# ebiggers/libdeflate

Hardware: NVIDIA H100
Metric: MB/s compress+decompress (batched 64 KiB chunks) (higher is better)
Workload: dtype u8

## Files before the change

### libdeflate_b200/csrc/deflate_block.cuh

```cuda
#pragma once

struct lz_group {
	u32 tid, lane, warp, gw, gt;
	__device__ __forceinline__ void sync() const
	{
		if (gt < LZ_THREADS) LDB_BAR_SYNC(LZ_BAR_P, gt);
		else __syncthreads();
	}
};

__constant__ u8 lz_precode_perm[DEFLATE_NUM_PRECODE_SYMS] = {16, 17, 18, 0, 8, 7, 9, 6, 10, 5, 11, 4, 12, 3, 13, 2, 14, 1, 15};

__device__ __forceinline__ u32 lz_static_litlen_len(u32 sym) { return sym < 144 ? 8 : (sym < 256 ? 9 : (sym < 280 ? 7 : 8)); }

__device__ __forceinline__ u32 lz_warp_incl_scan(u32 x, u32 lane)
{
	for (int o2 = 1; o2 < 32; o2 <<= 1) {
		const u32 t = __shfl_up_sync(LDB_FULL_MASK, x, o2);
		if (lane >= (u32)o2) x += t;
	}
	return x;
}

__device__ __forceinline__ u32 lz_group_excl_scan(const lz_group &g, u32 *escan, u32 x, u32 &total)
{
	const u32 incl = lz_warp_incl_scan(x, g.lane);
	if (g.lane == 31) escan[g.warp] = incl;
	g.sync();
	if (g.warp == 0) {
		const u32 y = g.lane < g.gw ? escan[g.lane] : 0;
		const u32 yi = lz_warp_incl_scan(y, g.lane);
		if (g.lane < g.gw) escan[32 + g.lane] = yi - y;
		if (g.lane == g.gw - 1) escan[64] = yi;
	}
	g.sync();
	total = escan[64];
	return escan[32 + g.warp] + (incl - x);
}

struct lz_out {
	u8 *out;
	size_t avail;
	u64 obit;
};

__device__ __forceinline__ void lz_stage_or(u32 *stage, u32 rel_bit, u64 bits, u32 nbits)
{
	if (!nbits) return;
	u32 w = rel_bit >> 5, sh = rel_bit & 31;
	atomicOr(&stage[w], (u32)(bits << sh));
	if (sh + nbits > 32) {
		u64 rest = bits >> (32 - sh);
		atomicOr(&stage[w + 1], (u32)rest);
		if (sh + nbits > 64) atomicOr(&stage[w + 2], (u32)(rest >> 32));
	}
}

__device__ __forceinline__ void lz_stage_reset(const lz_group &g, u32 *stage, const lz_out &o, const u32 *carry)
{
	for (u32 k = g.tid; k < LZ_STAGE_WORDS; k += g.gt) stage[k] = 0;
	g.sync();
	if (g.tid == 0) {
		u32 wv = 0;
		if (carry) {
			wv = *carry;
		} else {
			const u8 *wp = o.out + (o.obit >> 5) * 4;
			for (u32 k = 0; k < (u32)((o.obit >> 3) & 3); k++) wv |= (u32)(*(volatile const u8 *)(wp + k)) << (8 * k);
		}
		stage[0] = wv;
	}
	g.sync();
}

__device__ __forceinline__ void lz_stage_store(const lz_group &g, const u32 *stage, u8 *out, u64 w0, u64 end)
{
	const u64 begin = w0 * 4;
	for (u64 k = begin + g.tid; k < end; k += g.gt) {
		const u32 rel = (u32)(k - begin);
		out[k] = (u8)(stage[rel >> 2] >> (8 * (rel & 3)));
	}
}

__device__ __forceinline__ void lz_flush_words(const lz_out &o, const u32 *stage, u64 first_word, u32 nwords, u32 nthreads)
{
	if ((((uintptr_t)o.out) & 3) == 0) {
		u32 *dst = (u32 *)o.out + first_word;
		for (u32 i = threadIdx.x; i < nwords; i += nthreads) dst[i] = stage[i];
	} else {
		u8 *dst = o.out + first_word * 4;
		for (u32 i = threadIdx.x; i < nwords * 4; i += nthreads) dst[i] = (u8)(stage[i >> 2] >> (8 * (i & 3)));
	}
}

__device__ __forceinline__ void lz_huffman_merge(u32 *nodefreq, u16 *parent, u32 nused)
{
	const u32 INF = 0xffffffffu;
	u32 leaf = 0, inode = nused, nn = nused;
	u32 l0 = nodefreq[0], l1 = nused > 1 ? nodefreq[1] : INF;
	u32 n0 = INF, n1 = INF;
	while (nn < 2 * nused - 1) {
		u32 a, b, fa, fb;
		if (l0 <= n0) { a = leaf++; fa = l0; l0 = l1; l1 = leaf + 1 < nused ? nodefreq[leaf + 1] : INF; }
		else { a = inode++; fa = n0; n0 = n1; n1 = INF; }
		if (n0 == INF && inode < nn) n0 = nodefreq[inode];
		if (l0 <= n0) { b = leaf++; fb = l0; l0 = l1; l1 = leaf + 1 < nused ? nodefreq[leaf + 1] : INF; }
		else { b = inode++; fb = n0; n0 = n1; n1 = INF; }
		const u32 sum = fa + fb;
		nodefreq[nn] = sum;
		parent[a] = (u16)nn;
		parent[b] = (u16)nn;
		nn++;
		if (n0 == INF && inode < nn) n0 = inode == nn - 1 ? sum : nodefreq[inode];
		if (n1 == INF && inode + 1 < nn) n1 = inode + 1 == nn - 1 ? sum : nodefreq[inode + 1];
	}
}

#define LZ_SM_CNT    (LZ_SM_GEXIT + 256)
#define LZ_SM_PFREQ  (LZ_SM_GEXIT)
#define LZ_SM_PLENS  (LZ_SM_GEXIT + 128)
#define LZ_SM_PCODES (LZ_SM_GEXIT + 160)

__device__ __forceinline__ void lz_canonical_codes(const lz_group &g, u8 *sm)
{
	const u8 *lens = sm + LZ_SM_LENS;
	u16 *codes = (u16 *)(sm + LZ_SM_CODES);
	const u32 tid = g.tid;
	if (tid < 320) {
		const u32 l = lens[tid];
		u32 code = 0;
		if (l) {
			const u32 lo = tid < 288 ? 0 : 288;
			const u32 *cn = (u32 *)(sm + LZ_SM_CNT) + (tid < 288 ? 0 : 17);
			u32 first = 0;
			for (u32 k = 1; k < l; k++) first = (first + cn[k]) << 1;
			u32 same = 0;
			for (u32 t = lo; t < tid; t++) same += lens[t] == l;
			code = __brev(first + same) >> (32 - l);
		}
		codes[tid] = (u16)code;
	}
	g.sync();
}

__device__ __forceinline__ void lz_build_codes(const lz_group &g, u8 *sm)
{
	lz_vars *v = (lz_vars *)(sm + LZ_SM_VARS);
	u32 *freq = (u32 *)(sm + LZ_SM_FREQ);
	u8 *lens = sm + LZ_SM_LENS;
	u16 *hsorted = (u16 *)(sm + LZ_SM_R);
	u32 *hnodefreq = (u32 *)(sm + LZ_SM_R + 1024);
	u16 *hparent = (u16 *)(sm + LZ_SM_R + 1024 + 2304);
	u16 *osorted = (u16 *)(sm + LZ_SM_R + 4608);
	u32 *onodefreq = (u32 *)(sm + LZ_SM_R + 4608 + 128);
	u16 *oparent = (u16 *)(sm + LZ_SM_R + 4608 + 128 + 512);
	u32 *hcount = (u32 *)(sm + LZ_SM_CNT), *ocount = hcount + 17;
	const u32 tid = g.tid;
	const bool is_lit = tid < 288;
	const u32 lo = is_lit ? 0 : 288, hi = is_lit ? 288 : 320;
	if (tid == 0) { freq[256] = 1; v->nused_lit = 0; v->nused_off = 0; v->huff_over = 0; }
	if (tid < 34) hcount[tid] = 0;
	g.sync();
	u32 myrank = 0xffffffffu;
	if (tid < 320) {
		const u32 f = freq[tid];
		lens[tid] = 0;
		if (f) {
			u32 rank = 0;
			for (u32 t = lo; t < hi; t++) {
				u32 ft = freq[t];
				rank += (ft != 0) && (ft < f || (ft == f && t < tid));
			}
			myrank = rank;
			(is_lit ? hsorted : osorted)[rank] = (u16)(tid - lo);
			(is_lit ? hnodefreq : onodefreq)[rank] = f;
			atomicAdd(is_lit ? &v->nused_lit : &v->nused_off, 1u);
		}
	}
	g.sync();
	const u32 nused = is_lit ? v->nused_lit : v->nused_off;
	if (tid == 0 && nused >= 2) lz_huffman_merge(hnodefreq, hparent, nused);
	if (tid == 32) { const u32 nu = v->nused_off; if (nu >= 2) lz_huffman_merge(onodefreq, oparent, nu); }
	g.sync();
	if (tid < 320 && myrank != 0xffffffffu && nused >= 2) {
		const u16 *par = is_lit ? hparent : oparent;
		const u32 root = 2 * nused - 2;
		u32 node = myrank, d = 0;
		while (node != root && d <= 15) { node = par[node]; d++; }
		if (d > 15) { d = 15; v->huff_over = 1; }
		atomicAdd(&(is_lit ? hcount : ocount)[d], 1u);
	}
	g.sync();
	if ((tid == 0 || tid == 288) && nused < 2) {
		u8 *ln = lens + lo;
		u32 *cn = is_lit ? hcount : ocount;
		if (nused == 0) { ln[0] = 1; ln[1] = 1; }
		else { const u32 sy = (is_lit ? hsorted : osorted)[0]; ln[sy] = 1; ln[sy ? 0 : 1] = 1; }
		cn[1] = 2;
	}
	if ((tid == 0 || tid == 32) && v->huff_over) {
		u32 *cn = tid == 0 ? hcount : ocount;
		u32 kraft = 0;
		for (u32 l = 1; l <= 15; l++) kraft += cn[l] << (15 - l);
		while (kraft > (1u << 15)) {
			u32 l = 14;
			while (cn[l] == 0) l--;
			cn[l]--;
			cn[l + 1] += 2;
			cn[15]--;
			kraft -= 1;
		}
	}
	g.sync();
	if (tid < 320 && myrank != 0xffffffffu && nused >= 2) {
		const u32 *cn = is_lit ? hcount : ocount;
		u32 cum = 0, len = 1;
		for (u32 l = 15; l >= 1; l--) {
			cum += cn[l];
			if (myrank < cum) { len = l; break; }
		}
		lens[tid] = (u8)len;
	}
	g.sync();
	lz_canonical_codes(g, sm);
}

__device__ __forceinline__ void lz_precode(const lz_group &g, u8 *sm)
{
	lz_vars *v = (lz_vars *)(sm + LZ_SM_VARS);
	const u8 *lens = sm + LZ_SM_LENS;
	u16 *items = (u16 *)(sm + LZ_SM_ITEMS);
	u32 *escan = (u32 *)(sm + LZ_SM_ESCAN);
	u32 *pfreq_sm = (u32 *)(sm + LZ_SM_PFREQ);
	u8 *plens_sm = sm + LZ_SM_PLENS;
	u16 *pcodes_sm = (u16 *)(sm + LZ_SM_PCODES);
	const u32 tid = g.tid, lane = g.lane, warp = g.warp;
	if (tid == 0) {
		u32 hlit = 288;
		while (hlit > 257 && lens[hlit - 1] == 0) hlit--;
		v->hlit = hlit;
	}
	if (tid == 32) {
		u32 hdist = 32;
		while (hdist > 1 && lens[288 + hdist - 1] == 0) hdist--;
		v->hdist = hdist;
	}
	if (tid >= 64 && tid < 64 + 19) pfreq_sm[tid - 64] = 0;
	g.sync();
	{
		const u32 hlit = v->hlit, total = hlit + v->hdist;
		const u32 j = tid;
		const bool inb = j < total;
		const u32 val = inb ? (j < hlit ? lens[j] : lens[288 + j - hlit]) : 0xff;
		const u32 prv = (inb && j > 0) ? (j - 1 < hlit ? lens[j - 1] : lens[288 + j - 1 - hlit]) : 0xfe;
		const bool isstart = inb && val != prv;
		const u32 smask = __ballot_sync(LDB_FULL_MASK, isstart);
		if (lane == 0 && warp < 10) escan[66 + warp] = smask;
		g.sync();
		u32 run = 0, cnt = 0;
		if (isstart) {
			u32 nxt = total;
			u32 m = lane == 31 ? 0 : (smask & ~((2u << lane) - 1));
			if (m) nxt = warp * 32 + __ffs(m) - 1;
			else {
				for (u32 w = warp + 1; w < 10; w++) {
					u32 mm = escan[66 + w];
					if (mm) { nxt = w * 32 + __ffs(mm) - 1; break; }
				}
			}
			run = nxt - j;
			if (val == 0) {
				u32 rem = run % 138;
				cnt = run / 138 + (rem >= 3 ? 1 : rem);
			} else if (run >= 4) {
				u32 rem = (run - 1) % 6;
				cnt = 1 + (run - 1) / 6 + (rem >= 3 ? 1 : rem);
			} else cnt = run;
		}
		u32 ntot;
		const u32 off = lz_group_excl_scan(g, escan, cnt, ntot);
		if (isstart) {
			u32 ni = off;
			if (val == 0) {
				while (run >= 11) {
					u32 r = run < 138 ? run : 138;
					items[ni++] = (u16)(18 | ((r - 11) << 5));
					atomicAdd(&pfreq_sm[18], 1u);
					run -= r;
				}
				if (run >= 3) {
					items[ni++] = (u16)(17 | ((run - 3) << 5));
					atomicAdd(&pfreq_sm[17], 1u);
					run = 0;
				}
			} else if (run >= 4) {
				items[ni++] = (u16)val;
				atomicAdd(&pfreq_sm[val], 1u);
				run--;
				while (run >= 3) {
					u32 r = run < 6 ? run : 6;
					items[ni++] = (u16)(16 | ((r - 3) << 5));
					atomicAdd(&pfreq_sm[16], 1u);
					run -= r;
				}
			}
			if (run) atomicAdd(&pfreq_sm[val], run);
			while (run) { items[ni++] = (u16)val; run--; }
		}
		if (tid == 0) v->n_items = ntot;
	}
	g.sync();
	if (warp == 0) {
		u32 *pnodef = (u32 *)(sm + LZ_SM_GEXIT + 512);
		u16 *ppar = (u16 *)(sm + LZ_SM_GEXIT + 672);
		const u32 lt = (1u << lane) - 1;
		const u32 f = lane < 19 ? pfreq_sm[lane] : 0;
		const u32 usedm = __ballot_sync(LDB_FULL_MASK, f != 0);
		const u32 nused = __popc(usedm);
		u32 rank = 0;
		for (u32 t = 0; t < 19; t++) {
			const u32 ft = __shfl_sync(LDB_FULL_MASK, f, t);
			rank += (ft != 0) && (ft < f || (ft == f && t < lane));
		}
		if (f) pnodef[rank] = f;
		__syncwarp();
		if (lane == 0 && nused >= 2) lz_huffman_merge(pnodef, ppar, nused);
		__syncwarp();
		u32 d = 0;
		bool over = false;
		if (f && nused >= 2) {
			const u32 root = 2 * nused - 2;
			u32 node = rank;
			while (node != root && d <= 7) { node = ppar[node]; d++; }
			if (d > 7) { d = 7; over = true; }
		}
		u64 cn = 0;
		for (u32 l = 1; l <= 7; l++) cn |= (u64)__popc(__ballot_sync(LDB_FULL_MASK, d == l)) << (8 * l);
		if (__any_sync(LDB_FULL_MASK, over)) {
			u32 kraft = 0;
			for (u32 l = 1; l <= 7; l++) kraft += (u32)((cn >> (8 * l)) & 0xff) << (7 - l);
			while (kraft > (1u << 7)) {
				u32 l = 6;
				while (((cn >> (8 * l)) & 0xff) == 0) l--;
				cn -= (u64)1 << (8 * l);
				cn += (u64)2 << (8 * (l + 1));
				cn -= (u64)1 << (8 * 7);
				kraft -= 1;
			}
		}
		u32 len = 0;
		if (nused >= 2) {
			if (f) {
				u32 cum = 0;
				len = 1;
				for (u32 l = 7; l >= 1; l--) {
					cum += (u32)((cn >> (8 * l)) & 0xff);
					if (rank < cum) { len = l; break; }
				}
			}
		} else {
			const u32 sy = nused ? (u32)__ffs(usedm) - 1 : 0;
			len = (lane == sy || lane == (sy ? 0u : 1u)) ? 1 : 0;
			cn = (u64)2 << 8;
		}
		u32 first = 0;
		for (u32 k = 1; k < len; k++) first = (first + (u32)((cn >> (8 * k)) & 0xff)) << 1;
		const u32 samem = __match_any_sync(LDB_FULL_MASK, len);
		const u32 code = len ? __brev(first + __popc(samem & lt)) >> (32 - len) : 0;
		if (lane < 19) { plens_sm[lane] = (u8)len; pcodes_sm[lane] = (u16)code; }
		__syncwarp();
		const u32 nzm = __ballot_sync(LDB_FULL_MASK, lane < 19 && plens_sm[lz_precode_perm[lane < 19 ? lane : 0]] != 0);
		u32 hclen = nzm ? 32 - __clz(nzm) : 0;
		if (hclen < 4) hclen = 4;
		u32 cost = f * len + (lane == 16 ? 2 * f : lane == 17 ? 3 * f : lane == 18 ? 7 * f : 0);
		for (int o2 = 16; o2 > 0; o2 >>= 1) cost += __shfl_xor_sync(LDB_FULL_MASK, cost, o2);
		if (lane == 0) {
			v->cost_dyn = cost + 3 + 5 + 5 + 4 + 3 * hclen;
			v->hclen = hclen;
			v->cost_static = 3;
		}
	}
	g.sync();
}

#define LZ_NOFIT 0xffffffffu

__device__ __forceinline__ u32 lz_block_choose(const lz_group &g, u8 *sm, const lz_out &o, u32 blen, u32 tail)
{
	lz_vars *v = (lz_vars *)(sm + LZ_SM_VARS);
	const u32 *freq = (const u32 *)(sm + LZ_SM_FREQ);
	const u8 *lens = sm + LZ_SM_LENS;
	const u32 tid = g.tid;
	if (tid < 320) {
		u32 f = freq[tid];
		if (f) {
			u32 dyn = f * lens[tid];
			u32 extra = 0, st;
			if (tid < 288) {
				st = f * lz_static_litlen_len(tid);
				if (tid >= 257) extra = f * lz_len_extra_bits(tid - 257);
			} else {
				st = f * 5;
				extra = f * lz_off_extra_bits(tid - 288);
			}
			atomicAdd(&v->cost_dyn, dyn + extra);
			atomicAdd(&v->cost_static, st + extra);
		}
	}
	g.sync();
	const u32 cost_dyn = v->cost_dyn, cost_static = v->cost_static;
	const u32 bitoff = (u32)(o.obit & 7);
	const u32 stored_pieces = blen ? (blen + 65534) / 65535 : 1;
	const u64 cost_stored = (u64)(((bitoff + 3 + 7) & ~7u) - bitoff) + 32 + (u64)8 * blen + (u64)(stored_pieces - 1) * 40;
	u32 btype = DEFLATE_BLOCKTYPE_STORED;
	u64 best = cost_stored;
	if (cost_static < best) { best = cost_static; btype = DEFLATE_BLOCKTYPE_STATIC; }
	if (cost_dyn < best) { best = cost_dyn; btype = DEFLATE_BLOCKTYPE_DYNAMIC; }
	if ((o.obit + best + 7) / 8 + tail > o.avail) {
		if (tid == 0) v->failed = 1;
		g.sync();
		return LZ_NOFIT;
	}
	return btype;
}

__device__ __forceinline__ void lz_emit_stored(const lz_group &g, u8 *sm, lz_out &o, const u8 *src, u32 blen, bool fin)
{
	u32 *stage = (u32 *)(sm + LZ_SM_R);
	const u32 pieces = blen ? (blen + 65534) / 65535 : 1;
	u32 done = 0;
	for (u32 piece = 0; piece < pieces; piece++) {
		const u32 len = blen - done > 65535 ? 65535 : blen - done;
		const u64 w0 = o.obit >> 5;
		if (g.tid == 0) {
			lz_stage_or(stage, (u32)(o.obit - (w0 << 5)), fin && piece + 1 == pieces ? 1 : 0, 3);
			u64 ob = (o.obit + 3 + 7) & ~(u64)7;
			lz_stage_or(stage, (u32)(ob - (w0 << 5)), (u64)len | ((u64)(~len & 0xffff) << 16), 32);
		}
		o.obit = ((o.obit + 3 + 7) & ~(u64)7) + 32;
		g.sync();
		lz_stage_store(g, stage, o.out, w0, o.obit >> 3);
		g.sync();
		u8 *dst = o.out + (o.obit >> 3);
		for (u32 k = g.tid; k < len; k += g.gt) dst[k] = src[done + k];
		done += len;
		o.obit += (u64)len * 8;
		lz_stage_reset(g, stage, o, nullptr);
	}
}

__device__ __forceinline__ void lz_emit_huffman(const lz_group &g, u8 *sm, lz_out &o, const u32 *tokbuf, u32 ntok, u32 btype,
						bool fin)
{
	lz_vars *v = (lz_vars *)(sm + LZ_SM_VARS);
	u8 *lens = sm + LZ_SM_LENS;
	const u16 *codes = (const u16 *)(sm + LZ_SM_CODES);
	const u16 *items = (const u16 *)(sm + LZ_SM_ITEMS);
	u32 *escan = (u32 *)(sm + LZ_SM_ESCAN);
	u32 *stage = (u32 *)(sm + LZ_SM_R);
	const u32 tid = g.tid;
	if (btype == DEFLATE_BLOCKTYPE_STATIC) {
		if (tid < 320) lens[tid] = tid < 288 ? (u8)lz_static_litlen_len(tid) : 5;
		if (tid < 34) ((u32 *)(sm + LZ_SM_CNT))[tid] = tid == 7 ? 24 : (tid == 8 ? 152 : (tid == 9 ? 112 : (tid == 17 + 5 ? 32 : 0)));
		g.sync();
		lz_canonical_codes(g, sm);
	}
	u64 w0 = o.obit >> 5;
	u32 rel;
	{
		const u32 rb0 = (u32)(o.obit - (w0 << 5));
		u32 rb = rb0 + 3;
		if (tid == 0) lz_stage_or(stage, rb0, (fin ? 1 : 0) | (btype << 1), 3);
		if (btype == DEFLATE_BLOCKTYPE_DYNAMIC) {
			const u8 *plens_sm = sm + LZ_SM_PLENS;
			const u16 *pcodes_sm = (const u16 *)(sm + LZ_SM_PCODES);
			const u32 hclen = v->hclen, nit = v->n_items;
			if (tid == 0) lz_stage_or(stage, rb, (v->hlit - 257) | ((v->hdist - 1) << 5) | ((hclen - 4) << 10), 14);
			rb += 14;
			if (tid < hclen) lz_stage_or(stage, rb + 3 * tid, plens_sm[lz_precode_perm[tid]], 3);
			rb += 3 * hclen;
			u32 nb = 0, bits = 0;
			if (tid < nit) {
				const u32 it = items[tid], sym = it & 31, ex = it >> 5;
				const u32 pl = plens_sm[sym];
				const u32 eb = sym == 16 ? 2 : (sym == 17 ? 3 : (sym == 18 ? 7 : 0));
				bits = pcodes_sm[sym] | (ex << pl);
				nb = pl + eb;
			}
			u32 hbits;
			const u32 hoff = lz_group_excl_scan(g, escan, nb, hbits);
			lz_stage_or(stage, rb + hoff, bits, nb);
			rb += hbits;
		}
		rel = rb;
	}
	g.sync();
	const u32 tpt = LZ_TPT(g.gt);
	for (u32 t0 = 0; t0 <= ntok; t0 += g.gt * tpt) {
		u32 mybits[2] = {};
		u64 myval[2] = {};
#pragma unroll
		for (u32 r = 0; r < 2; r++) {
			u32 ti = r < tpt ? t0 + tid * tpt + r : 0xffffffffu;
			if (ti < ntok) {
				u32 tk = tokbuf[ti];
				if (tk & 0x80000000u) {
					u32 len = ((tk >> 15) & 0x1ff) + 3, off = (tk & 0x7fff) + 1;
					u32 ls = lz_len_slot(len), os = lz_off_slot(off);
					u32 nb = lens[257 + ls];
					u64 val = codes[257 + ls];
					u32 leb = lz_len_extra_bits(ls);
					val |= (u64)(len - lz_len_base(ls)) << nb;
					nb += leb;
					val |= (u64)codes[288 + os] << nb;
					nb += lens[288 + os];
					u32 oeb = lz_off_extra_bits(os);
					val |= (u64)(off - lz_off_base(os)) << nb;
					nb += oeb;
					mybits[r] = nb;
					myval[r] = val;
				} else {
					mybits[r] = lens[tk];
					myval[r] = codes[tk];
				}
			} else if (ti == ntok) {
				mybits[r] = lens[256];
				myval[r] = codes[256];
			}
		}
		u32 round_bits;
		u32 bitpos = rel + lz_group_excl_scan(g, escan, mybits[0] + mybits[1], round_bits);
#pragma unroll
		for (u32 r = 0; r < 2; r++) {
			lz_stage_or(stage, bitpos, myval[r], mybits[r]);
			bitpos += mybits[r];
		}
		g.sync();
		rel += round_bits;
		u32 full = rel >> 5;
		if (full) {
			lz_flush_words(o, stage, w0, full, g.gt);
			g.sync();
			u32 carry = stage[full];
			g.sync();
			for (u32 k = tid; k <= full && k < LZ_STAGE_WORDS; k += g.gt) stage[k] = 0;
			g.sync();
			if (tid == 0) stage[0] = carry;
			w0 += full;
			rel &= 31;
			g.sync();
		}
	}
	o.obit = (w0 << 5) + rel;
}

__device__ __forceinline__ void lz_finish(const lz_group &g, u8 *sm, const ldb_deflate_args &a, size_t c, const lz_out &o,
					  bool nonfinal)
{
	lz_vars *v = (lz_vars *)(sm + LZ_SM_VARS);
	u32 *stage = (u32 *)(sm + LZ_SM_R);
	if (v->failed) {
		if (g.tid == 0) a.out_nbytes[c] = 0;
		return;
	}
	const u64 w0 = o.obit >> 5;
	lz_stage_reset(g, stage, o, &v->carry);
	u64 ob;
	if (!nonfinal) {
		const u32 trailer = ldb_trl_bytes(a.format);
		ob = (o.obit + 7) & ~(u64)7;
		if (g.tid == 0 && trailer) {
			u8 t[8];
			def_write_trailer(t, a.format, a.checksums ? a.checksums[c] : 0, a.in_nbytes[c]);
			for (u32 k = 0; k < trailer; k++) lz_stage_or(stage, (u32)(ob - (w0 << 5)) + 8 * k, t[k], 8);
		}
		ob += (u64)trailer * 8;
	} else {
		ob = (o.obit + 3 + 7) & ~(u64)7;
		if (g.tid == 0) lz_stage_or(stage, (u32)(ob - (w0 << 5)), 0xffff0000u, 32);
		ob += 32;
	}
	g.sync();
	lz_stage_store(g, stage, o.out, w0, ob >> 3);
	if (g.tid == 0) a.out_nbytes[c] = (size_t)(ob >> 3);
}
```

### libdeflate_b200/csrc/deflate_lz_kernel.cuh

```cuda
#pragma once

#define LZ_THREADS   1024
#define LZ_WARPS     (LZ_THREADS / 32)
#define LZ_PASS      16384
#define LZ_BLOCK_PASSES 2
#define LZ_NWIN      (LZ_PASS / 32)
#define LZ_NSL_BITS  5
#define LZ_NSL       (1 << LZ_NSL_BITS)
#define LZ_SEG       16384
#define LZ_RING      65536
#define LZ_HASH_BITS 13
#define LZ_WIN       32768
#define LZ_LOOKAHEAD 512
#define LZ_MAX_DIST  (LZ_WIN - LZ_LOOKAHEAD)
#define LZ_TOKCAP    (LZ_BLOCK_PASSES * LZ_PASS + 64)
#define LZ_STAGE_WORDS 2048
#define LZ_TPT(gt)     ((gt) > 512 ? 1u : 2u)
#define LZ_GROUP_PARSE     {12, 10, 8, 8, 8, 5, 16, 16, 16}
#define LZ_GROUP_FLUSH     12
#define LZ_GROUP_HAND      10
#define LZ_GROUP_MIN_PARSE 4
#define LZ_GROUP_MIN_FLUSH 10
#define LZ_GROUP_MAX       28
#define LZ_BAR_P     1
#define LZ_BAR_S     2
#define LZ_BAR_H     3
#define LZ_PF        4
#define LZ_RUN_SHORT 16
#ifndef LZ_SPEC_ROUNDS
#define LZ_SPEC_ROUNDS 4
#endif
static_assert(LZ_SPEC_ROUNDS >= 1 && LZ_SPEC_ROUNDS <= 14, "round statistic buckets");
static_assert(LZ_GROUP_MIN_PARSE >= 1 && LZ_GROUP_MIN_FLUSH * 32 >= 320 && LZ_GROUP_MAX < LZ_WARPS, "group size bounds");
static_assert(LZ_GROUP_FLUSH >= LZ_GROUP_MIN_FLUSH && LZ_GROUP_FLUSH <= LZ_GROUP_MAX && LZ_GROUP_HAND >= LZ_GROUP_MIN_FLUSH &&
	      LZ_GROUP_HAND <= LZ_GROUP_MAX, "default group sizes");

#define LZ_SM_RING   0
#define LZ_SM_NEXT   (LZ_SM_RING + LZ_RING)
#define LZ_SM_HEAD   (LZ_SM_NEXT + 2 * 65536)
#define LZ_SM_R      (LZ_SM_HEAD + 2 * (1 << LZ_HASH_BITS))
#define LZ_SM_VIS    (LZ_SM_R)
#define LZ_SM_TOKOFF (LZ_SM_R + 4096)
#define LZ_SM_ENTRY  (LZ_SM_R + 8320)
#define LZ_SM_ESCAN  (LZ_SM_R + 9344)
#define LZ_SM_GEXIT  (LZ_SM_R + 9728)
#define LZ_SM_ITEMS  (LZ_SM_R + 12288)
#define LZ_SM_FREQ   (LZ_SM_ITEMS + 1024)
#define LZ_SM_LENS   (LZ_SM_FREQ + 4 * 320)
#define LZ_SM_CODES  (LZ_SM_LENS + 320)
#define LZ_SM_VARS   (LZ_SM_CODES + 2 * 320)
#define LZ_SM_BYTES  (LZ_SM_VARS + 256)

#define LZ_BLOCK_POS (LZ_BLOCK_PASSES * LZ_PASS)
#define LZ_OPT_K     8
#define LZ_DP_SEG    2048
#define LZ_GS_RES    0
#define LZ_GS_TOK    (LZ_GS_RES + 4 * LZ_BLOCK_POS)
#define LZ_GS_COST   (LZ_GS_TOK + 4 * LZ_TOKCAP)
#define LZ_GS_MLIST  (LZ_GS_COST + 4 * (LZ_BLOCK_POS + 320))
#define LZ_GS_BYTES  (LZ_GS_MLIST + 4 * LZ_BLOCK_POS * LZ_OPT_K)
#define LZ_FAR4_DIST  1024
#define LZ_COST_INF  0x3fffffu

struct lz_vars {
	unsigned long long mbar;
	u32 chunk;
	u32 tok_count;
	u32 parse_entry;
	u32 cost_dyn, cost_static;
	u32 hlit, hdist, hclen;
	u32 n_items;
	u32 run_counter;
	u32 min_len;
	u32 far4_dist;
	u32 used_lits[8];
	u32 carry;
	u32 nused_lit, nused_off;
	u32 huff_over;
	u32 obs_blk[8], obs_next[8];
	u32 end_block;
	u32 failed;
	u32 obit_lo, obit_hi;
	u32 blk_begin, blk_entry, blk_passes;
	u32 pre_lens_packed[3];
	u32 tma_phase;
	u32 dict, nonfinal;
	u32 spec_last;
	u32 spec_first;
	u32 prefetched;
	u32 nx_min_len, nx_far4;
};
static_assert(sizeof(lz_vars) <= 256, "lz_vars fits its shared-memory slot");

struct lz_params {
	int depth, nice, lazy;
	int opt_iters;
};

__device__ __forceinline__ lz_params lz_level_params(int level)
{
	switch (level) {
	case 1: return {2, 16, 0, 0};
	case 2: return {4, 24, 0, 0};
	case 3: return {8, 32, 0, 0};
	case 4: return {12, 48, 0, 0};
	case 5: return {12, 48, 1, 0};
	case 6: return {24, 96, 1, 0};
	case 7: return {48, 160, 1, 0};
	case 8: return {96, 258, 2, 0};
	case 9: return {200, 258, 2, 0};
	case 10: return {48, 96, 1, 2};
	case 11: return {96, 160, 1, 3};
	default: return {200, 258, 1, 5};
	}
}

__device__ __forceinline__ u32 lz_choose_min_len(u32 num_used_literals, u32 depth)
{
	u32 m;
	if (num_used_literals < 6) m = 9;
	else if (num_used_literals < 8) m = 8;
	else if (num_used_literals < 10) m = 7;
	else if (num_used_literals < 16) m = 6;
	else if (num_used_literals < 45) m = 5;
	else m = 4;
	if (depth < 16) {
		u32 cap = depth < 5 ? 4 : (depth < 10 ? 5 : 7);
		if (m > cap) m = cap;
	}
	return m;
}

__device__ __forceinline__ u32 lz_ld32(const u8 *ring, u32 pos)
{
	u32 a = pos & (LZ_RING - 1);
	const u32 *w = (const u32 *)ring;
	u32 lo = w[a >> 2];
	u32 hi = w[((a + 4) & (LZ_RING - 1)) >> 2];
	return __funnelshift_r(lo, hi, (a & 3) * 8);
}
__device__ __forceinline__ u32 lz_ld8(const u8 *ring, u32 pos) { return ring[pos & (LZ_RING - 1)]; }
__device__ __forceinline__ u32 lz_hash(u32 v) { return (v * 0x1E35A7BDu) >> (32 - LZ_HASH_BITS); }

template <typename Bar>
__device__ __forceinline__ void lz_load_segment(u8 *sm, lz_vars *v, const u8 *in, u32 from, u32 to, u32 gt, u32 gn, Bar bar)
{
	u8 *ring = sm + LZ_SM_RING;
	u32 len = to - from;
	u32 bulk = (((uintptr_t)(in + from) & 15) == 0) ? (len & ~15u) : 0;
	bar();
#ifndef LDB_EMU
	if (bulk) {
		u32 mbar = (u32)__cvta_generic_to_shared(&v->mbar);
		if (gt == 0) {
			u32 dst = (u32)__cvta_generic_to_shared(ring + (from & (LZ_RING - 1)));
			asm volatile("fence.proxy.async.shared::cta;" ::: "memory");
			asm volatile("mbarrier.arrive.expect_tx.shared::cta.b64 _, [%0], %1;" ::"r"(mbar), "r"(bulk) : "memory");
			asm volatile("cp.async.bulk.shared::cluster.global.mbarrier::complete_tx::bytes [%0], [%1], %2, [%3];"
				     ::"r"(dst), "l"(in + from), "r"(bulk), "r"(mbar) : "memory");
		}
		u32 phase = v->tma_phase;
		u32 done = 0;
		while (!done) {
			asm volatile("{\n\t.reg .pred p;\n\tmbarrier.try_wait.parity.shared::cta.b64 p, [%1], %2;\n\tselp.u32 %0, 1, 0, p;\n\t}"
				     : "=r"(done) : "r"(mbar), "r"(phase) : "memory");
		}
	}
#else
	for (u32 i = gt; i < bulk; i += gn) ring[(from + i) & (LZ_RING - 1)] = in[from + i];
#endif
	for (u32 i = bulk + gt; i < len; i += gn) ring[(from + i) & (LZ_RING - 1)] = in[from + i];
	bar();
	if (bulk && gt == 0) v->tma_phase ^= 1;
	bar();
}

__device__ __forceinline__ u32 lz_len_slot(u32 len)
{
	if (len < 11) return len - 3;
	if (len == 258) return 28;
	u32 l = len - 3;
	u32 eb = 29 - __clz(l);
	return 4 * eb + 4 + ((l >> eb) & 3);
}
__device__ __forceinline__ u32 lz_len_extra_bits(u32 slot) { return (slot < 8 || slot == 28) ? 0 : (slot - 4) >> 2; }
__device__ __forceinline__ u32 lz_len_base(u32 slot) { return slot < 8 ? 3 + slot : (slot == 28 ? 258 : 3 + ((4 + (slot & 3)) << ((slot - 4) >> 2))); }
__device__ __forceinline__ u32 lz_off_slot(u32 off)
{
	if (off < 5) return off - 1;
	u32 o = off - 1;
	u32 eb = 30 - __clz(o);
	return 2 * eb + 2 + ((o >> eb) & 1);
}
__device__ __forceinline__ u32 lz_off_extra_bits(u32 slot) { return slot < 4 ? 0 : (slot - 2) >> 1; }
__device__ __forceinline__ u32 lz_off_base(u32 slot) { return slot < 4 ? 1 + slot : 1 + ((2 + (slot & 1)) << ((slot - 2) >> 1)); }

#include "deflate_block.cuh"

#ifdef LZ_TIMING
#include <stdio.h>
#define LZ_TSLOTS 30
__device__ unsigned long long ldb_lz_timing[2][LZ_TSLOTS];
#define LZ_TCLK (tid == 0 || tid == LZ_THREADS - 32)
#define LZ_T(k) do { if (LZ_TCLK) { long long t_ = clock64(); tacc[k] += t_ - tlast; tlast = t_; } } while (0)
#define LZ_TSPAN_BEGIN() do { if (LZ_TCLK) tspan = clock64(); } while (0)
#define LZ_TSPAN_END(k) do { if (LZ_TCLK) tacc[k] += clock64() - tspan; } while (0)
#define LZ_TSPLIT_BEGIN() do { if (LZ_TCLK) tsplit = clock64(); } while (0)
#define LZ_TSPLIT_BUSY() do { if (tid == 0) tbusy = clock64() - tsplit; } while (0)
#define LZ_TJOIN_BEGIN() do { if (LZ_TCLK) tjoin = clock64(); } while (0)
#define LZ_TSPLIT_END(split, kind) do { if ((split) && LZ_TCLK) { const long long t_ = clock64(); const int k_ = (kind); \
	tacc[18 + k_] += tbusy; tacc[21 + k_] += t_ - tjoin; tacc[24 + k_] += 1; tacc[27 + k_] += t_ - tsplit; } } while (0)
#else
#define LZ_T(k) do { } while (0)
#define LZ_TSPAN_BEGIN() do { } while (0)
#define LZ_TSPAN_END(k) do { } while (0)
#define LZ_TSPLIT_BEGIN() do { } while (0)
#define LZ_TSPLIT_BUSY() do { } while (0)
#define LZ_TJOIN_BEGIN() do { } while (0)
#define LZ_TSPLIT_END(split, kind) do { } while (0)
#endif

#ifdef LZ_SPEC_STATS
__device__ unsigned long long ldb_lz_spec_rounds[16];
extern "C" __attribute__((visibility("default"))) void ldb_lz_spec_stats(unsigned long long *out, int reset)
{
#ifdef LDB_EMU
	for (int i = 0; i < 16; i++) { out[i] = ldb_lz_spec_rounds[i]; if (reset) ldb_lz_spec_rounds[i] = 0; }
#else
	unsigned long long z[16] = {};
	cudaDeviceSynchronize();
	cudaMemcpyFromSymbol(out, ldb_lz_spec_rounds, sizeof(z));
	if (reset) cudaMemcpyToSymbol(ldb_lz_spec_rounds, z, sizeof(z));
#endif
}
#endif

template <int NBITS>
__device__ __forceinline__ u32 lz_same_key_mask(u32 key, bool valid)
{
	u32 m = __ballot_sync(LDB_FULL_MASK, valid);
#pragma unroll
	for (int b = 0; b < NBITS; b++) {
		const u32 bal = __ballot_sync(LDB_FULL_MASK, (key >> b) & 1);
		m &= ((key >> b) & 1) ? bal : ~bal;
	}
	return m;
}

template <typename Bar, typename Decided>
__device__ __forceinline__ void lz_insert_pass_par(const u8 *ring, u16 *head, u16 *nextt, u32 *cmat,
						   u32 b0, u32 pend, u32 n, u32 tid, u32 lane, u32 warp, u32 gw, Bar bar,
						   bool decide, Decided decided
#ifdef LZ_TIMING
						   , long long *tacc, long long &tlast
#endif
						   )
{
	static_assert((LZ_WARPS * LZ_NSL + 2 * LZ_NSL) * 4 <= 8192, "count matrix fits the start of region R");
	u32 *sbase = cmat + LZ_WARPS * LZ_NSL, *stot = sbase + LZ_NSL;
	const u32 lt = (1u << lane) - 1;
	const u32 LB = (b0 + LZ_PASS) & 0xffff;
	const u32 ntiles = (pend - b0 + 31) >> 5, tpw = (ntiles + gw - 1) / gw;
	const u32 r0 = b0 + warp * tpw * 32;
	const u32 r1 = r0 + tpw * 32 < pend ? r0 + tpw * 32 : pend;
	for (u32 i = tid; i < LZ_WARPS * LZ_NSL + 2 * LZ_NSL; i += 32 * gw) cmat[i] = 0;
	bar();
	for (u32 p = r0 + lane; p < r1; p += 32) {
		const u32 hv = p + 4 <= n ? lz_hash(lz_ld32(ring, p)) : 0xffffu;
		nextt[p & 0xffff] = (u16)hv;
		if (hv != 0xffffu) atomicAdd(&cmat[warp * LZ_NSL + (hv >> (LZ_HASH_BITS - LZ_NSL_BITS))], 1u);
	}
	bar();
	LZ_T(12);
	if (decide && tid == 32 * (gw - 1)) decided();
	if (warp == 0) {
		u32 run = 0;
		if (lane < LZ_NSL)
			for (u32 w = 0; w < gw; w++) {
				const u32 c = cmat[w * LZ_NSL + lane];
				cmat[w * LZ_NSL + lane] = run;
				run += c;
			}
		u32 incl = run;
		for (int o2 = 1; o2 < LZ_NSL; o2 <<= 1) {
			const u32 t = __shfl_up_sync(LDB_FULL_MASK, incl, o2);
			if (lane >= (u32)o2) incl += t;
		}
		if (lane < LZ_NSL) { sbase[lane] = incl - run; stot[lane] = run; }
	}
	bar();
	for (u32 t = 0; t < tpw; t++) {
		const u32 p = r0 + 32 * t + lane;
		const u32 hv = p < r1 ? nextt[p & 0xffff] : 0xffffu;
		const bool valid = hv != 0xffffu;
		const u32 sl = hv >> (LZ_HASH_BITS - LZ_NSL_BITS);
		const u32 m = lz_same_key_mask<LZ_NSL_BITS>(sl, valid);
		const u32 cur = valid ? cmat[warp * LZ_NSL + sl] : 0;
		__syncwarp();
		if (valid) {
			nextt[LB + sbase[sl] + cur + __popc(m & lt)] = (u16)p;
			if ((m & lt) == 0) cmat[warp * LZ_NSL + sl] = cur + __popc(m);
		}
		__syncwarp();
	}
	bar();
	LZ_T(13);
	for (u32 s = warp; s < LZ_NSL; s += gw) {
		const u32 cnt = stot[s];
		const u16 *mylist = nextt + LB + sbase[s];
		u32 p16n = lane < cnt ? mylist[lane] : 0;
		u32 hn = lane < cnt ? nextt[p16n] : 0;
		for (u32 b = 0; b < cnt; b += 32) {
			const bool valid = b + lane < cnt;
			const u32 p16 = p16n;
			const u32 h = valid ? hn : 0;
			if (b + 32 + lane < cnt) {
				p16n = mylist[b + 32 + lane];
				hn = nextt[p16n];
			}
			const u32 old_head = valid ? head[h] : 0;
// ... 853 lines not shown
```

Before: 16250.

## Parallelize Huffman code build, block cost, and bit emission with warp primitives

Replaces the O(n) per-thread serial loops in canonical code assignment and frequency ranking with warp match/ballot counts and vectorized key comparisons over packed (freq, symbol) keys. Block cost accumulation now uses warp reductions followed by one atomic per warp, instead of an atomic per symbol. The emit loop picks a variable tokens-per-thread count, up to four, bounded by the stage capacity. The flush clears stage words inline, which removes several group barriers per flush. The risks are extra register pressure from the larger per-thread arrays, and shared-memory aliasing of the new key and word-count scratch regions.

```diff
diff --git a/libdeflate_b200/csrc/deflate_block.cuh b/libdeflate_b200/csrc/deflate_block.cuh
--- a/libdeflate_b200/csrc/deflate_block.cuh
+++ b/libdeflate_b200/csrc/deflate_block.cuh
@@ -82,14 +82,18 @@
 	}
 }
 
-__device__ __forceinline__ void lz_flush_words(const lz_out &o, const u32 *stage, u64 first_word, u32 nwords, u32 nthreads)
-{
-	if ((((uintptr_t)o.out) & 3) == 0) {
-		u32 *dst = (u32 *)o.out + first_word;
-		for (u32 i = threadIdx.x; i < nwords; i += nthreads) dst[i] = stage[i];
-	} else {
-		u8 *dst = o.out + first_word * 4;
-		for (u32 i = threadIdx.x; i < nwords * 4; i += nthreads) dst[i] = (u8)(stage[i >> 2] >> (8 * (i & 3)));
+__device__ __forceinline__ void lz_flush_words(const lz_out &o, u32 *stage, u64 first_word, u32 nwords, u32 nthreads)
+{
+	const bool aligned = (((uintptr_t)o.out) & 3) == 0;
+	for (u32 i = threadIdx.x; i < nwords; i += nthreads) {
+		const u32 w = stage[i];
+		if (aligned) {
+			((u32 *)o.out)[first_word + i] = w;
+		} else {
+			u8 *d = o.out + (first_word + i) * 4;
+			for (u32 k = 0; k < 4; k++) d[k] = (u8)(w >> (8 * k));
+		}
+		stage[i] = 0;
 	}
 }
 
@@ -120,22 +124,35 @@
 #define LZ_SM_PFREQ  (LZ_SM_GEXIT)
 #define LZ_SM_PLENS  (LZ_SM_GEXIT + 128)
 #define LZ_SM_PCODES (LZ_SM_GEXIT + 160)
+#define LZ_SM_WCNT   (LZ_SM_GEXIT + 768)
 
 __device__ __forceinline__ void lz_canonical_codes(const lz_group &g, u8 *sm)
 {
 	const u8 *lens = sm + LZ_SM_LENS;
 	u16 *codes = (u16 *)(sm + LZ_SM_CODES);
-	const u32 tid = g.tid;
+	u32 *wcnt = (u32 *)(sm + LZ_SM_WCNT);
+	const u32 tid = g.tid, lane = g.lane, warp = g.warp;
+	u32 l = 0, samem = 0;
 	if (tid < 320) {
-		const u32 l = lens[tid];
+		l = lens[tid];
+		samem = __match_any_sync(LDB_FULL_MASK, l);
+		u32 mine = 0;
+		for (u32 k = 1; k <= 15; k++) {
+			const u32 c = __popc(__ballot_sync(LDB_FULL_MASK, l == k));
+			if (lane == k) mine = c;
+		}
+		if (warp < 9 && lane < 16) wcnt[warp * 16 + lane] = mine;
+	}
+	g.sync();
+	if (tid < 320) {
 		u32 code = 0;
 		if (l) {
-			const u32 lo = tid < 288 ? 0 : 288;
 			const u32 *cn = (u32 *)(sm + LZ_SM_CNT) + (tid < 288 ? 0 : 17);
 			u32 first = 0;
 			for (u32 k = 1; k < l; k++) first = (first + cn[k]) << 1;
-			u32 same = 0;
-			for (u32 t = lo; t < tid; t++) same += lens[t] == l;
+			u32 same = __popc(samem & ((1u << lane) - 1));
+			if (warp < 9)
+				for (u32 w = 0; w < warp; w++) same += wcnt[w * 16 + l];
 			code = __brev(first + same) >> (32 - l);
 		}
 		codes[tid] = (u16)code;
@@ -155,26 +172,35 @@
 	u32 *onodefreq = (u32 *)(sm + LZ_SM_R + 4608 + 128);
 	u16 *oparent = (u16 *)(sm + LZ_SM_R + 4608 + 128 + 512);
 	u32 *hcount = (u32 *)(sm + LZ_SM_CNT), *ocount = hcount + 17;
+	u32 *key = (u32 *)(sm + LZ_SM_R + 5632);
 	const u32 tid = g.tid;
 	const bool is_lit = tid < 288;
 	const u32 lo = is_lit ? 0 : 288, hi = is_lit ? 288 : 320;
-	if (tid == 0) { freq[256] = 1; v->nused_lit = 0; v->nused_off = 0; v->huff_over = 0; }
+	if (tid == 0) { v->nused_lit = 0; v->nused_off = 0; v->huff_over = 0; }
 	if (tid < 34) hcount[tid] = 0;
+	u32 f = 0;
+	if (tid < 320) {
+		f = tid == 256 ? 1 : freq[tid];
+		if (tid == 256) freq[256] = 1;
+		key[tid] = f ? (f << 9) | (tid - lo) : 0xffffffffu;
+		lens[tid] = 0;
+	}
 	g.sync();
 	u32 myrank = 0xffffffffu;
 	if (tid < 320) {
-		const u32 f = freq[tid];
-		lens[tid] = 0;
+		const u32 nu = __popc(__ballot_sync(LDB_FULL_MASK, f != 0));
+		if (g.lane == 0 && nu) atomicAdd(is_lit ? &v->nused_lit : &v->nused_off, nu);
 		if (f) {
+			const u32 k = key[tid];
+			const uint4 *kq = (const uint4 *)(key + lo);
 			u32 rank = 0;
-			for (u32 t = lo; t < hi; t++) {
-				u32 ft = freq[t];
-				rank += (ft != 0) && (ft < f || (ft == f && t < tid));
+			for (u32 q = 0; q < (hi - lo) / 4; q++) {
+				const uint4 kk = kq[q];
+				rank += (kk.x < k) + (kk.y < k) + (kk.z < k) + (kk.w < k);
 			}
 			myrank = rank;
 			(is_lit ? hsorted : osorted)[rank] = (u16)(tid - lo);
 			(is_lit ? hnodefreq : onodefreq)[rank] = f;
-			atomicAdd(is_lit ? &v->nused_lit : &v->nused_off, 1u);
 		}
 	}
 	g.sync();
@@ -392,19 +418,20 @@
 	const u8 *lens = sm + LZ_SM_LENS;
 	const u32 tid = g.tid;
 	if (tid < 320) {
-		u32 f = freq[tid];
-		if (f) {
-			u32 dyn = f * lens[tid];
-			u32 extra = 0, st;
-			if (tid < 288) {
-				st = f * lz_static_litlen_len(tid);
-				if (tid >= 257) extra = f * lz_len_extra_bits(tid - 257);
-			} else {
-				st = f * 5;
-				extra = f * lz_off_extra_bits(tid - 288);
-			}
-			atomicAdd(&v->cost_dyn, dyn + extra);
-			atomicAdd(&v->cost_static, st + extra);
+		const u32 f = freq[tid];
+		u32 extra = 0, st;
+		if (tid < 288) {
+			st = f * lz_static_litlen_len(tid);
+			if (tid >= 257) extra = f * lz_len_extra_bits(tid - 257);
+		} else {
+			st = f * 5;
+			extra = f * lz_off_extra_bits(tid - 288);
+		}
+		const u32 dyn = __reduce_add_sync(LDB_FULL_MASK, f * lens[tid] + extra);
+		st = __reduce_add_sync(LDB_FULL_MASK, st + extra);
+		if (g.lane == 0) {
+			atomicAdd(&v->cost_dyn, dyn);
+			atomicAdd(&v->cost_static, st);
 		}
 	}
 	g.sync();
@@ -495,12 +522,13 @@
 		rel = rb;
 	}
 	g.sync();
-	const u32 tpt = LZ_TPT(g.gt);
-	for (u32 t0 = 0; t0 <= ntok; t0 += g.gt * tpt) {
-		u32 mybits[2] = {};
-		u64 myval[2] = {};
+	for (u32 t0 = 0; t0 <= ntok; ) {
+		u32 tpt = ((LZ_STAGE_WORDS - 2) * 32 - rel) / (48 * g.gt);
+		if (tpt > LZ_EMIT_TPT) tpt = LZ_EMIT_TPT;
+		u32 mybits[LZ_EMIT_TPT] = {}, sumbits = 0;
+		u64 myval[LZ_EMIT_TPT] = {};
 #pragma unroll
-		for (u32 r = 0; r < 2; r++) {
+		for (u32 r = 0; r < LZ_EMIT_TPT; r++) {
 			u32 ti = r < tpt ? t0 + tid * tpt + r : 0xffffffffu;
 			if (ti < ntok) {
 				u32 tk = tokbuf[ti];
@@ -527,29 +555,27 @@
 				mybits[r] = lens[256];
 				myval[r] = codes[256];
 			}
+			sumbits += mybits[r];
 		}
 		u32 round_bits;
-		u32 bitpos = rel + lz_group_excl_scan(g, escan, mybits[0] + mybits[1], round_bits);
+		u32 bitpos = rel + lz_group_excl_scan(g, escan, sumbits, round_bits);
 #pragma unroll
-		for (u32 r = 0; r < 2; r++) {
+		for (u32 r = 0; r < LZ_EMIT_TPT; r++) {
 			lz_stage_or(stage, bitpos, myval[r], mybits[r]);
 			bitpos += mybits[r];
 		}
 		g.sync();
 		rel += round_bits;
-		u32 full = rel >> 5;
+		const u32 full = rel >> 5;
 		if (full) {
+			const u32 carry = tid == 0 ? stage[full] : 0;
 			lz_flush_words(o, stage, w0, full, g.gt);
-			g.sync();
-			u32 carry = stage[full];
-			g.sync();
-			for (u32 k = tid; k <= full && k < LZ_STAGE_WORDS; k += g.gt) stage[k] = 0;
-			g.sync();
-			if (tid == 0) stage[0] = carry;
+			if (tid == 0) { stage[full] = 0; stage[0] = carry; }
 			w0 += full;
 			rel &= 31;
 			g.sync();
 		}
+		t0 += g.gt * tpt;
 	}
 	o.obit = (w0 << 5) + rel;
 }
diff --git a/libdeflate_b200/csrc/deflate_lz_kernel.cuh b/libdeflate_b200/csrc/deflate_lz_kernel.cuh
--- a/libdeflate_b200/csrc/deflate_lz_kernel.cuh
+++ b/libdeflate_b200/csrc/deflate_lz_kernel.cuh
@@ -15,7 +15,7 @@
 #define LZ_MAX_DIST  (LZ_WIN - LZ_LOOKAHEAD)
 #define LZ_TOKCAP    (LZ_BLOCK_PASSES * LZ_PASS + 64)
 #define LZ_STAGE_WORDS 2048
-#define LZ_TPT(gt)     ((gt) > 512 ? 1u : 2u)
+#define LZ_EMIT_TPT    4
 #define LZ_GROUP_PARSE     {12, 10, 8, 8, 8, 5, 16, 16, 16}
 #define LZ_GROUP_FLUSH     12
 #define LZ_GROUP_HAND      10
```

New measurement: 16330 (median of 6 runs). Within noise of the previous version (+0.5%).
